# TMElyralab/MuseV

Measured on NVIDIA H100. Metric: denoised frames/sec at 512x512, 16-frame window, 20 DDIM steps, higher is better.
Workload: dtype f16 (fp32 accumulate)

## Files before the change

include/musev_b200.h:

```cpp
#ifndef MUSEV_B200_H_
#define MUSEV_B200_H_

#include <stdint.h>

#ifdef __cplusplus
extern "C" {
#endif

#define MVB_OK 0
#define MVB_ERR_INVALID (-1)
#define MVB_ERR_CUDA (-2)
#define MVB_ERR_STATE (-3)

const char* mvb_last_error(void);
int mvb_version(void);

typedef struct mvb_conv_gemm_desc {
  const void* a0; int c0; long long a0_stride_w, a0_stride_h, a0_stride_n;
  const void* a1; int c1; long long a1_stride_w, a1_stride_h, a1_stride_n;
  int W, H, NF;
  int ntaps; int8_t dy[9]; int8_t dx[9];
  const void* weight; int N;
  void* out; long long ldc;
  const float* bias;
// ... 98 lines not shown
#define MVB_MAX_REFER 16
typedef struct mvb_unet_args {
  const void* sample; int sample_is_f32;
  int B, T, H, W;
  float timestep;
  const void* encoder_hidden_states; int ehs_is_f32; int n_text;
  int has_sample_index;
  int n_vis_cond, vis_cond_first;
  float sample_frame_rate;
  const void* vision_clip_emb; int clip_is_f32; int n_clip; float ip_adapter_scale;
  int n_refer;
  const void* refer_embs[MVB_MAX_REFER]; int refer_t[MVB_MAX_REFER], refer_h[MVB_MAX_REFER], refer_w[MVB_MAX_REFER];
  const void* mid_refer_emb; int mid_refer_t, mid_refer_h, mid_refer_w;
  int refer_is_f32;
  int n_down_residuals;
  const void* down_residuals[MVB_MAX_REFER];
  const void* mid_residual; int residual_is_f32;
  int skip_temporal_layers;
  void* out; int out_is_f32;
  const void* pose_guider_emb; int pose_is_f32;
} mvb_unet_args;

int mvb_create(const mvb_config* cfg, int device, mvb_handle** out);
void mvb_destroy(mvb_handle* h);
int mvb_load_weight(mvb_handle* h, const char* name, const void* device_ptr, int is_f32, const long long* shape, int ndim);
typedef struct mvb_named_tensor {
  const char* name;
  const void* device_ptr;
  int is_f32;
  int ndim;
// ... 78 lines not shown
```

musev_b200/_capi.py:

```python
from __future__ import annotations

import ctypes as C
import hashlib
import os
from types import SimpleNamespace
from typing import Callable, Dict, Iterable, Optional, Sequence, Tuple

import torch
import torch.distributed as dist

from .build import LIB_PATH
from .context import assign_windows

_lib = None


class MvbError(RuntimeError):
    pass


class ConvGemmDesc(C.Structure):
    _fields_ = [
        ("a0", C.c_void_p), ("c0", C.c_int),
        ("a0_stride_w", C.c_longlong), ("a0_stride_h", C.c_longlong), ("a0_stride_n", C.c_longlong),
# ... 40 lines not shown
class MvbUnetArgs(C.Structure):
    _fields_ = [
        ("sample", C.c_void_p), ("sample_is_f32", C.c_int),
        ("B", C.c_int), ("T", C.c_int), ("H", C.c_int), ("W", C.c_int),
        ("timestep", C.c_float),
        ("encoder_hidden_states", C.c_void_p), ("ehs_is_f32", C.c_int), ("n_text", C.c_int),
        ("has_sample_index", C.c_int),
        ("n_vis_cond", C.c_int), ("vis_cond_first", C.c_int),
        ("sample_frame_rate", C.c_float),
        ("vision_clip_emb", C.c_void_p), ("clip_is_f32", C.c_int), ("n_clip", C.c_int), ("ip_adapter_scale", C.c_float),
        ("n_refer", C.c_int),
        ("refer_embs", C.c_void_p * MAX_REFER), ("refer_t", C.c_int * MAX_REFER), ("refer_h", C.c_int * MAX_REFER),
        ("refer_w", C.c_int * MAX_REFER),
        ("mid_refer_emb", C.c_void_p), ("mid_refer_t", C.c_int), ("mid_refer_h", C.c_int), ("mid_refer_w", C.c_int),
        ("refer_is_f32", C.c_int),
        ("n_down_residuals", C.c_int), ("down_residuals", C.c_void_p * MAX_REFER),
        ("mid_residual", C.c_void_p), ("residual_is_f32", C.c_int),
        ("skip_temporal_layers", C.c_int),
        ("out", C.c_void_p), ("out_is_f32", C.c_int),
        ("pose_guider_emb", C.c_void_p), ("pose_is_f32", C.c_int),
    ]


class MvbNamedTensor(C.Structure):
    _fields_ = [("name", C.c_char_p), ("device_ptr", C.c_void_p), ("is_f32", C.c_int), ("ndim", C.c_int),
                ("shape", C.c_longlong * 5)]


MAX_OUT = 13


# ... 375 lines not shown
```

musev_b200/csrc/capi_ops.cu:

```cuda
#include <cuda_runtime.h>
#include <stdint.h>
#include <stdio.h>
#include <string.h>

#include "../../include/musev_b200.h"
#include "attention.cuh"
#include "cond_embed.cuh"
#include "conv_gemm.cuh"
#include "ops.cuh"

using namespace mvb;

static thread_local char g_err[512] = "";

static int fail(const char* what, cudaError_t e) {
  snprintf(g_err, sizeof(g_err), "%s: %s", what ? what : "error", e == cudaSuccess ? "invalid argument" : cudaGetErrorString(e));
  return e == cudaSuccess ? MVB_ERR_INVALID : MVB_ERR_CUDA;
}

static int sm_count() {
  static int n = 0;
  if (!n) {
    int dev = 0;
    if (cudaGetDevice(&dev) != cudaSuccess) return 132;
    if (cudaDeviceGetAttribute(&n, cudaDevAttrMultiProcessorCount, dev) != cudaSuccess || n <= 0) n = 132;
  }
  return n;
}

extern "C" {

const char* mvb_last_error(void) { return g_err; }

int mvb_version(void) { return 6; }

int mvb_op_conv_gemm(const mvb_conv_gemm_desc* d, void* stream) {
  if (!d || !d->a0 || !d->weight || !d->out) return fail("mvb_op_conv_gemm: null pointer", cudaSuccess);
  ASource a0{(const __half*)d->a0, d->c0, d->a0_stride_w, d->a0_stride_h, d->a0_stride_n};
  ASource a1{(const __half*)d->a1, d->c1, d->a1_stride_w, d->a1_stride_h, d->a1_stride_n};
  Epilogue ep;
  ep.out = (__half*)d->out; ep.ldc = d->ldc; ep.bias = d->bias; ep.rowadd = d->rowadd;
  ep.rows_per_group = d->rows_per_group; ep.ld_rowadd = d->ld_rowadd; ep.res = (const __half*)d->residual;
  ep.ld_res = d->ld_res; ep.alpha = d->alpha; ep.beta = d->beta; ep.geglu = d->geglu; ep.act = d->act; ep.out_f32 = d->out_f32;
  const char* err = nullptr;
  if (d->stride2) {
    cudaError_t e2 = launch_conv_s2((cudaStream_t)stream, (const __half*)d->a0, d->c0, d->W, d->H, d->NF,
                                    (const __half*)d->weight, d->N, ep, sm_count(), &err, d->stride2);
    if (e2 != cudaSuccess) return fail(err, e2);
    return MVB_OK;
// ... 48 lines not shown
int mvb_op_temporal_attention(const void* qkv, int ld, int B, int T, int HW, int heads, int d, int dp, float scale,
                              void* out, int ldo, void* stream) {
  cudaError_t e = temporal_attention((cudaStream_t)stream, (const __half*)qkv, ld, B, T, HW, heads, d, dp, scale,
                                     (__half*)out, ldo);
  if (e == cudaErrorInvalidValue)
    return fail("mvb_op_temporal_attention: needs 1 <= T <= 32, d a multiple of 8, dp in {16, 32, 48, 64, 80, 96, 160} "
                "with dp >= d, ld and ldo multiples of 8", cudaSuccess);
  if (e != cudaSuccess) return fail("mvb_op_temporal_attention", e);
  return MVB_OK;
}

int mvb_op_groupnorm(const void* x0, int c0, const void* x1, int c1, int NF, int HW, int groups, int frames_per_stat,
                     float eps, const float* gamma, const float* beta, int silu, void* y, float* scratch, void* stream) {
  int chunks = 0;
  cudaError_t e = gn_stats((cudaStream_t)stream, (const __half*)x0, c0, (const __half*)x1, c1, NF, HW, groups, scratch,
                           &chunks);
  if (e == cudaSuccess)
    e = gn_apply((cudaStream_t)stream, (const __half*)x0, c0, (const __half*)x1, c1, NF, HW, groups, scratch, chunks,
                 frames_per_stat, eps, gamma, beta, silu, (__half*)y);
  if (e != cudaSuccess) return fail("mvb_op_groupnorm", e == cudaErrorInvalidValue ? cudaSuccess : e);
  return MVB_OK;
}

int mvb_op_groupnorm_fused(const void* x0, int c0, const void* x1, int c1, int NF, int HW, int groups, int frames_per_stat,
                           float eps, const float* gamma, const float* beta, int silu, void* y, float* scratch,
                           unsigned int* barrier_word, unsigned int* arrivals, void* stream) {
  if (!barrier_word || !arrivals) return fail("mvb_op_groupnorm_fused: null barrier word", cudaSuccess);
  int dev = 0, sms = 132;
  cudaGetDevice(&dev);
  cudaDeviceGetAttribute(&sms, cudaDevAttrMultiProcessorCount, dev);
  cudaError_t e = gn_fused((cudaStream_t)stream, (const __half*)x0, c0, (const __half*)x1, c1, NF, HW, groups, scratch,
                           frames_per_stat, eps, gamma, beta, silu, (__half*)y, sms, barrier_word, arrivals);
  if (e != cudaSuccess) return fail("mvb_op_groupnorm_fused", e == cudaErrorInvalidValue ? cudaSuccess : e);
  return MVB_OK;
}

int mvb_op_layernorm(const void* x, long long M, int C, float eps, const float* gamma, const float* beta, void* y,
                     void* stream) {
  cudaError_t e = layernorm((cudaStream_t)stream, (const __half*)x, M, C, eps, gamma, beta, (__half*)y);
  if (e != cudaSuccess) return fail("mvb_op_layernorm", e == cudaErrorInvalidValue ? cudaSuccess : e);
  return MVB_OK;
}

int mvb_fuse_cfg_ddim(const float* eps_sum, const float* counter, const void* latents_in, void* latents_out,
                      int is_f32, int B, int C, int T, int HW, int cfg, float guidance_scale, float alpha_prod_t,
                      float alpha_prod_t_prev, int prediction_type, float clip_range, int use_clipped_model_output,
                      float std_dev_t, const float* variance_noise, float* eps_out, float* x0_out, void* stream) {
// ... 54 lines not shown
```

musev_b200/csrc/engine_fwd.cuh:

```cuda
#pragma once
#include <math.h>
#include <stdio.h>

#include <string>

#include "attention.cuh"
#include "conv_gemm.cuh"
#include "engine.cuh"
#include "ops.cuh"

namespace mvb {

inline constexpr const char* kNullArg = "null pointer argument";

struct Engine::Fwd {
  Engine* E;
  Arena* ar;
  cudaStream_t s;
  bool dry;
  int B, T, H, W, NF;
  int heads;
  int groups;
  float gn_eps;
  float* gn_part = nullptr;
  const float* temb_table = nullptr;
  const float* femb_table = nullptr;
  int temb_ld = 0, femb_ld = 0;
  struct Cond {
    const __half* enc = nullptr;
    int n_text = 0;
    const __half* clip = nullptr;
    int n_clip = 0;
    float ip_adapter_scale = 0.f;
    int n_vis_cond = 0, vis_cond_first = 0;
    int refer_is_f32 = 0;
  } cond;
  bool skip_temporal;
  bool ok = true;

  Fwd(Engine* e, Arena& arena, cudaStream_t st, int B_, int T_, int H_, int W_, bool skip_temporal_layers, int groups_,
      float gn_eps_)
      : E(e), ar(&arena), s(st), dry(arena.dry), B(B_), T(T_), H(H_), W(W_), NF(B_ * T_), heads(e->heads_), groups(groups_),
        gn_eps(gn_eps_), skip_temporal(skip_temporal_layers) {
    if (!dry) E->taps_.clear();
    if (groups) gn_part = alloc_f((long long)NF * (kGnMaxChunks + 1) * groups * 2);
  }

  bool fail(const char* what, cudaError_t e) {
    if (ok) {
      char buf[400];
      snprintf(buf, sizeof(buf), "%s: %s", what ? what : "error", e == cudaSuccess ? "failed" : cudaGetErrorString(e));
      E->err_ = buf;
    }
    ok = false;
    return false;
  }
  __half* alloc_h(long long rows, int C) {
    void* p = ar->alloc((size_t)rows * C * sizeof(__half));
    if (!p) fail("workspace too small", cudaSuccess);
    return (__half*)p;
  }
  float* alloc_f(long long n) {
    void* p = ar->alloc((size_t)n * sizeof(float));
    if (!p) fail("workspace too small", cudaSuccess);
    return (float*)p;
  }
  void tap(const std::string& name, const __half* p, long long rows, int C) {
    if (!dry) E->taps_.push_back({name, p, rows, C});
  }
  size_t mark() const { return ar->off; }
  void release(size_t m) { ar->off = m; }

  void gemm_img(const ASource& a0, const ASource* a1, int Wd, int Hd, int NFd, int ntaps, const int8_t* dy,
                const int8_t* dx, const Mat& m, Epilogue ep, bool use_bias = true) {
    if (!ok || dry) return;
    if (use_bias && !ep.bias) ep.bias = m.bias;
    const char* err = nullptr;
    cudaError_t e = launch_conv_gemm(s, a0, a1, Wd, Hd, NFd, ntaps, dy, dx, m.w, m.N, ep, E->num_sms_, &err);
    if (e != cudaSuccess) fail(err, e);
  }
  void gemm(const __half* x, long long M, int K, const Mat& m, Epilogue ep, bool use_bias = true) {
    static const int8_t z = 0;
    ASource a0{x, K, (long long)K, (long long)K * M, (long long)K * M};
// ... 9 lines not shown
  void conv1x1(const __half* x0, int C0, const __half* x1, int C1, long long M, const Mat& m, Epilogue ep) {
    static const int8_t z = 0;
    ASource a0{x0, C0, (long long)C0, (long long)C0 * M, (long long)C0 * M};
    ASource a1{x1, C1, (long long)C1, (long long)C1 * M, (long long)C1 * M};
    gemm_img(a0, x1 ? &a1 : nullptr, (int)M, 1, 1, 1, &z, &z, m, ep);
  }
  void tconv(const __half* x, int C, int HW, const Mat& m, Epilogue ep) {
    static const int8_t dy[3] = {-1, 0, 1}, dx[3] = {0, 0, 0};
    ASource a0{x, C, (long long)C, (long long)C * HW, (long long)C * HW * T};
    gemm_img(a0, nullptr, HW, T, B, 3, dy, dx, m, ep);
  }
  void gn(const __half* x0, int C0, const __half* x1, int C1, int HW, int fps, float eps, const Norm& n, int silu,
          __half* y) {
    if (!gn_part) { fail("groupnorm: the forward reserved no scratch", cudaSuccess); return; }
    if (!ok || dry) return;
    if (E->gn_fused_) {
      cudaError_t e = gn_fused(s, x0, C0, x1, C1, NF, HW, groups, gn_part, fps, eps, n.g, n.b, silu, y,
                               E->num_sms_, E->gn_counter_dev_, &E->gn_base_);
      if (e != cudaSuccess) fail("groupnorm (fused)", e);
      return;
    }
    int chunks = 0;
    cudaError_t e = gn_stats(s, x0, C0, x1, C1, NF, HW, groups, gn_part, &chunks);
    if (e == cudaSuccess)
      e = gn_apply(s, x0, C0, x1, C1, NF, HW, groups, gn_part, chunks, fps, eps, n.g, n.b, silu, y);
    if (e != cudaSuccess) fail("groupnorm", e);
  }
  void ln(const __half* x, long long M, int C, float eps, const Norm& n, __half* y) {
    if (!ok || dry) return;
    cudaError_t e = layernorm(s, x, M, C, eps, n.g, n.b, y);
    if (e != cudaSuccess) fail("layernorm", e);
  }
  void attn(const AttnArgs& aa) {
    if (!ok || dry) return;
    const char* err = nullptr;
    cudaError_t e = launch_attention(s, aa, &err);
    if (e != cudaSuccess) fail(err, e);
  }
// ... 112 lines not shown
  }
  void feed_forward(const TBlock& b, __half* h, long long M, int C, __half* nbuf) {
    const size_t mk = mark();
    ln(h, M, C, E->ln_eps13_, b.n3, nbuf);
    __half* ff = alloc_h(M, 4 * C);
    Epilogue e1;
    e1.out = ff; e1.ldc = 4 * C; e1.geglu = 1;
    gemm(nbuf, M, C, b.ff1, e1);
    Epilogue e2;
    e2.out = h; e2.ldc = C; e2.res = h; e2.ld_res = C;
    gemm(ff, M, 4 * C, b.ff2, e2);
    release(mk);
  }
  __half* spatial(const SpatialT& st, const __half* x, int HW) {
    const int C = st.C, Hh = heads, d = C / Hh, dp = pad16(d), hd = Hh * dp;
    const long long M = (long long)NF * HW;
    __half* out = alloc_h(M, C);
    const size_t mk = mark();
    __half* nbuf = alloc_h(M, C);
    __half* h = alloc_h(M, C);
    gn(x, C, nullptr, 0, HW, 1, 1e-6f, st.norm, 0, nbuf);
    { Epilogue ep; ep.out = h; ep.ldc = C; gemm(nbuf, M, C, st.proj_in, ep); }
    const TBlock& b = st.blk;
    {
      const size_t mk2 = mark();
      ln(h, M, C, E->ln_eps13_, b.n1, nbuf);
      __half* qkv = alloc_h(M, 3 * hd);
      { Epilogue ep; ep.out = qkv; ep.ldc = 3 * hd; gemm(nbuf, M, C, b.qkv1, ep, b.qkv1.bias != nullptr); }
      __half* ao = alloc_h(M, C);
      AttnArgs aa{};
      aa.v_ones_col = b.qkv1.bias != nullptr;
// ... 5 lines not shown
        aa.nseg = 2;
        aa.seg[1] = AttnSegment{qkv + hd, qkv + 2 * hd, 3 * hd, M, cond.n_vis_cond * HW, T, (long long)T * HW,
                                (long long)cond.vis_cond_first * HW};
      }
      aa.out = ao; aa.ldo = C; aa.out_scale = 1.f;
      attn(aa);
      Epilogue ep; ep.out = h; ep.ldc = C; ep.res = h; ep.ld_res = C;
      gemm(ao, M, C, b.out1, ep);
      release(mk2);
    }
    {
      const size_t mk2 = mark();
      ln(h, M, C, 1e-5f, b.n2, nbuf);
      __half* q = alloc_h(M, hd);
      { Epilogue ep; ep.out = q; ep.ldc = hd; gemm(nbuf, M, C, b.q2, ep, false); }
      const long long Mt = (long long)B * cond.n_text;
      __half* kv = alloc_h(Mt, 2 * hd);
      { Epilogue ep; ep.out = kv; ep.ldc = 2 * hd; gemm(cond.enc, Mt, b.kv2.K, b.kv2, ep, b.kv2.bias != nullptr); }
      __half* ao = alloc_h(M, C);
      AttnArgs aa{};
      aa.v_ones_col = b.kv2.bias != nullptr;
      aa.q = q; aa.ldq = hd; aa.NF = NF; aa.Nq = HW; aa.heads = Hh; aa.d = d; aa.dp = dp;
      aa.scale = 1.f / sqrtf((float)d);
      aa.nseg = 1;
      aa.seg[0] = AttnSegment{kv, kv + hd, 2 * hd, Mt, cond.n_text, T, cond.n_text, 0};
      aa.out = ao; aa.ldo = C; aa.out_scale = 1.f;
      attn(aa);
      if (b.has_ip && cond.clip && cond.ip_adapter_scale > 0.f) {
        const long long Mc = (long long)B * cond.n_clip;
        __half* kvi = alloc_h(Mc, 2 * hd);
// ... 66 lines not shown
    AttnArgs aa{};
    aa.q = qkv; aa.ldq = 3 * hd; aa.NF = NF; aa.Nq = HW; aa.heads = Hh; aa.d = d; aa.dp = dp;
    aa.scale = 1.f / sqrtf((float)d);
    aa.nseg = 2;
    aa.v_ones_col = r.qkv.bias != nullptr;
    aa.seg[0] = AttnSegment{kvr, kvr + hd, 2 * hd, Mr, nref, T, nref, 0};
    aa.seg[1] = AttnSegment{qkv + hd, qkv + 2 * hd, 3 * hd, M, HW, 1, HW, 0};
    aa.out = ao; aa.ldo = C; aa.out_scale = 1.f;
    attn(aa);
    Epilogue ep; ep.out = out; ep.ldc = C; ep.res = x; ep.ld_res = C;
    gemm(ao, M, C, r.out, ep);
    release(mk);
    return out;
  }
  __half* refer_tokens(const void* map, int C, int t, int h, int w) {
    __half* tok = alloc_h((long long)B * t * h * w, C);
    if (ok && !dry) {
      cudaError_t e = ncthw_to_tokens(s, map, cond.refer_is_f32, B, C, t, h * w, tok, C, 1.f);
      if (e != cudaSuccess) fail("refer tokens", e);
    }
    return tok;
  }
};

}
```

musev_b200/csrc/engine_unet.cu:

```cuda
#include "engine_fwd.cuh"

namespace mvb {

bool unet_config_ok(const mvb_config* cfg) {
  if (cfg->num_blocks < 1 || cfg->num_blocks > 4 || cfg->heads < 1 || cfg->norm_num_groups < 1) return false;
  for (int i = 0; i < cfg->num_blocks; ++i) {
    const int c = cfg->block_out_channels[i];
    if (c % 64 || c % cfg->heads || (c / cfg->heads) % 8 || c % cfg->norm_num_groups) return false;
  }
  return cfg->cross_attention_dim % 64 == 0 && cfg->in_channels * 9 <= 64;
}

void Engine::build_unet() {
  const mvb_config& c = cfg_;
  UNetWeights& w = model_.emplace<UNetWeights>();
  const int nb = c.num_blocks;
  const int c0 = c.block_out_channels[0], temb = 4 * c0;
  int n_res_c = 0, n_tt_c = 0;
  {
    int ch = c0;
    for (int i = 0; i < nb; ++i) {
      ch = c.block_out_channels[i];
      n_res_c += c.layers_per_block * ch;
      if (i != nb - 1) n_tt_c += c.layers_per_block * ch;
// ... 84 lines not shown
  w.norm_out = make_norm("conv_norm_out", c0);
  w.conv_out = make_mat(16, 9 * c0, true);
  reg_conv_cols("conv_out.weight", w.conv_out, 16, c.out_channels, c0, 9);
  reg_vec("conv_out.bias", w.conv_out.bias, 16, c.out_channels);
}

bool Engine::run_unet(const mvb_unet_args& a, Arena& ar, cudaStream_t s) {
  const mvb_config& c = cfg_;
  const UNetWeights& w = std::get<UNetWeights>(model_);
  const int nb = c.num_blocks, c0 = c.block_out_channels[0], temb = 4 * c0;
  const int B = a.B, T = a.T, NF = a.B * a.T;
  if (a.H % (1 << (nb - 1)) || a.W % (1 << (nb - 1))) { err_ = "H and W must be divisible by 2^(num_blocks-1)"; return false; }
  if (T > 32) { err_ = "at most 32 frames per window (temporal attention kernel)"; return false; }
  if (B < 1 || B > 64 || a.n_vis_cond > 64) { err_ = "batch (incl. CFG) must be in 1..64 and at most 64 vision-condition frames"; return false; }
  if (a.n_vis_cond < 0 || a.vis_cond_first < 0 || a.vis_cond_first + a.n_vis_cond > T) { err_ = "bad vision condition index range"; return false; }
  if (c.need_refer_emb && a.n_refer != 0) {
    int expect = 1;
    for (int i = 0; i < nb; ++i) expect += c.layers_per_block + (i == nb - 1 ? 0 : 1);
    if (a.n_refer != expect) { err_ = "down_block_refer_embs: wrong number of maps"; return false; }
  }
  Fwd f(this, ar, s, B, T, a.H, a.W, a.skip_temporal_layers != 0, c.norm_num_groups, c.norm_eps);

  __half* temb_rows = f.alloc_h(NF, temb);
  __half* femb_rows = f.alloc_h(NF, temb);
  float* temb_table = f.alloc_f((long long)NF * w.temb.rows);
  float* femb_table = f.alloc_f((long long)NF * w.femb.rows);
  f.temb_table = temb_table; f.femb_table = femb_table;
  f.temb_ld = w.temb.rows; f.femb_ld = w.femb.rows;
  {
    const size_t mk = f.mark();
// ... 32 lines not shown
  if (!ar.dry && f.ok) {
    cudaError_t e = ncthw_to_tokens(s, a.encoder_hidden_states, a.ehs_is_f32, 1, 1, 1, B * a.n_text * X, enc, 1, 1.f);
    if (e != cudaSuccess) f.fail("encoder_hidden_states convert", e);
  }
  if (c.ip_adapter_cross_attn && a.vision_clip_emb && a.n_clip > 0) {
    clip = f.alloc_h((long long)B * a.n_clip, X);
    if (!ar.dry && f.ok) {
      cudaError_t e = ncthw_to_tokens(s, a.vision_clip_emb, a.clip_is_f32, 1, 1, 1, B * a.n_clip * X, clip, 1, 1.f);
      if (e != cudaSuccess) f.fail("vision_clip_emb convert", e);
    }
  }
  Fwd::Cond& cd = f.cond;
  cd.enc = enc; cd.n_text = a.n_text; cd.clip = clip; cd.n_clip = a.n_clip; cd.ip_adapter_scale = a.ip_adapter_scale;
  if (c.need_t2i_ip_adapter) { cd.n_vis_cond = a.n_vis_cond; cd.vis_cond_first = a.vis_cond_first; } cd.refer_is_f32 = a.refer_is_f32;

  int Hc = a.H, Wc = a.W;
  const long long M = (long long)NF * Hc * Wc;
  __half* x = f.alloc_h(M, c0);
  f.conv_in(x, a.sample, a.sample_is_f32, c.in_channels, w.conv_in, a.pose_guider_emb, a.pose_is_f32, "conv_in inputs");
  f.tap("conv_in", x, M, c0);
  if (w.has_tin) { x = f.temporal(w.tin, x, Hc * Wc); f.tap("transformer_in", x, M, c0); }
  const bool use_ref = c.need_refer_emb && a.n_refer > 0;
  if (use_ref) {
    __half* tok = f.refer_tokens(a.refer_embs[0], c0, a.refer_t[0], a.refer_h[0], a.refer_w[0]);
    x = f.refer_fuse(w.first_ref, x, Hc * Wc, tok, a.refer_t[0] * a.refer_h[0] * a.refer_w[0]);
    f.tap("first_refer", x, M, c0);
  }
  struct Skip { __half* p; int C, H, W; };
  std::vector<Skip> skips;
  skips.push_back({x, c0, Hc, Wc});
  int ch = c0;
  for (int i = 0; i < nb; ++i) {
    const bool final = i == nb - 1;
    const Block& blk = w.down[i];
    const int num_block = c.layers_per_block + (final ? 0 : 1);
    const int ref_start = 1 + num_block * i;
    for (int j = 0; j < c.layers_per_block; ++j) {
      const Layer& L = blk.layers[j];
      const std::string pn = "down_blocks." + std::to_string(i);
      const long long Ml = (long long)NF * Hc * Wc;
      x = f.resnet(L.res, x, ch, nullptr, 0, Hc, Wc);
      ch = L.res.C;
      f.tap(pn + ".resnets." + std::to_string(j), x, Ml, ch);
      x = f.temp_conv(L.tc, x, Hc * Wc);
      f.tap(pn + ".temp_convs." + std::to_string(j), x, Ml, ch);
      if (L.has_attn) {
        x = f.spatial(L.st, x, Hc * Wc);
        f.tap(pn + ".attentions." + std::to_string(j), x, Ml, ch);
        x = f.temporal(L.tt, x, Hc * Wc);
        f.tap(pn + ".temp_attentions." + std::to_string(j), x, Ml, ch);
      }
      if (use_ref) {
        const int ri = ref_start + j;
        if (ri >= a.n_refer) { err_ = "refer emb index out of range"; return false; }
        __half* tok = f.refer_tokens(a.refer_embs[ri], ch, a.refer_t[ri], a.refer_h[ri], a.refer_w[ri]);
        x = f.refer_fuse(L.ref, x, Hc * Wc, tok, a.refer_t[ri] * a.refer_h[ri] * a.refer_w[ri]);
        f.tap(pn + ".refer_emb_attns." + std::to_string(j), x, Ml, ch);
      }
      skips.push_back({x, ch, Hc, Wc});
    }
    if (!final) {
      x = f.downsample(x, ch, Hc, Wc, blk.sampler, 1);
      Hc /= 2; Wc /= 2;
      if (use_ref) {
        const int ri = ref_start + c.layers_per_block;
        __half* tok = f.refer_tokens(a.refer_embs[ri], ch, a.refer_t[ri], a.refer_h[ri], a.refer_w[ri]);
        x = f.refer_fuse(blk.ref_down, x, Hc * Wc, tok, a.refer_t[ri] * a.refer_h[ri] * a.refer_w[ri]);
      }
      f.tap("down_blocks." + std::to_string(i) + ".down", x, (long long)NF * Hc * Wc, ch);
      skips.push_back({x, ch, Hc, Wc});
    }
  }
  x = f.resnet(w.mid_res[0], x, ch, nullptr, 0, Hc, Wc);
  x = f.temp_conv(w.mid_tc[0], x, Hc * Wc);
  x = f.spatial(w.mid_st, x, Hc * Wc);
  x = f.temporal(w.mid_tt, x, Hc * Wc);
  x = f.resnet(w.mid_res[1], x, ch, nullptr, 0, Hc, Wc);
  x = f.temp_conv(w.mid_tc[1], x, Hc * Wc);
  f.tap("mid", x, (long long)NF * Hc * Wc, ch);
  if (c.need_refer_emb && a.mid_refer_emb) {
    __half* tok = f.refer_tokens(a.mid_refer_emb, ch, a.mid_refer_t, a.mid_refer_h, a.mid_refer_w);
    x = f.refer_fuse(w.mid_ref, x, Hc * Wc, tok, a.mid_refer_t * a.mid_refer_h * a.mid_refer_w);
  }
  if (a.n_down_residuals > 0) {
    if (a.n_down_residuals != (int)skips.size()) { err_ = "down_block_additional_residuals: wrong count"; return false; }
// ... 57 lines not shown
```

musev_b200/csrc/ops.cu:

```cuda
#include "ops.cuh"

#include <math.h>

#include <type_traits>

#include "stats.cuh"

namespace mvb {

__device__ __forceinline__ float silu_f(float x) {
  float e, r;
  asm("ex2.approx.ftz.f32 %0, %1;" : "=f"(e) : "f"(x * -1.4426950408889634f));
  asm("rcp.approx.ftz.f32 %0, %1;" : "=f"(r) : "f"(1.f + e));
  return x * r;
}

struct alignas(16) Half8 {
  __half2 h[4];
};
__device__ __forceinline__ Half8 ld_half8(const __half* p) {
  Half8 r;
  *reinterpret_cast<uint4*>(&r) = __ldg(reinterpret_cast<const uint4*>(p));
  return r;
}
// ... 82 lines not shown
      }
    }
    float* dst = part + ((size_t)f * chunks + chunk) * 2 * G + 2 * g;
    dst[0] = mean;
    dst[1] = m2;
  }
}

__global__ void __launch_bounds__(256, 8)
gn_stats_kernel(const __half* __restrict__ x0, int C0, const __half* __restrict__ x1, int C1, int HW, int G,
                float* __restrict__ part) {
  extern __shared__ float2 spair[];
  gn_stats_unit(x0, C0, x1, C1, HW, G, part, gridDim.y - 1 - blockIdx.y, blockIdx.x, gridDim.x, spair);
}

cudaError_t gn_stats(cudaStream_t s, const __half* x0, int C0, const __half* x1, int C1, int NF, int HW, int G,
                     float* part, int* chunks_out) {
  ProfScope prof(s, KC_GROUPNORM);
  const int C = C0 + (x1 ? C1 : 0);
  if (!x1) C1 = 0;
  if ((C0 % 8) || (C1 % 8) || (C % G) || ((C / G) % 2)) return cudaErrorInvalidValue;
  const int threads = 256;
  int chunks = (8 * 132) / NF;
  const int maxc = HW / 32 > 0 ? HW / 32 : 1;
  if (chunks > maxc) chunks = maxc;
  if (chunks > kGnMaxChunks) chunks = kGnMaxChunks;
  if (chunks < 1) chunks = 1;
  *chunks_out = chunks;
  const int cols = (C / 8) < threads ? (C / 8) : threads;
  const size_t smem = (size_t)(threads / cols) * (C / 2) * sizeof(float2);
  gn_stats_kernel<<<dim3(chunks, NF), threads, smem, s>>>(x0, C0, x1, C1, HW, G, part);
  return cudaGetLastError();
}

__device__ __forceinline__ void gn_finalize_unit(const float* __restrict__ part, int chunks, int fps, int G, int HW, int cpg, float eps,
                                                 float* __restrict__ stats, int sg, int g, int lane) {
  float n = 0.f, mean = 0.f, m2 = 0.f;
  for (int i = lane; i < fps * chunks; i += 32) {
    const int chunk = i % chunks;
    const int pix = (int)(((long long)HW * (chunk + 1)) / chunks) - (int)(((long long)HW * chunk) / chunks);
    const float2 pp = *reinterpret_cast<const float2*>(part + ((size_t)sg * fps * chunks + i) * 2 * G + 2 * g);
    chan_merge(n, mean, m2, (float)pix * (float)cpg, pp.x, pp.y);
// ... 194 lines not shown
  int threads = 256;
  if (vecs <= 256 && (256 % vecs) != 0) threads = (256 / vecs) * vecs;
  if (threads < 64) threads = 256;
  const int rows_per_pass = threads / (vecs < threads ? vecs : threads) > 0 ? threads / (vecs < threads ? vecs : threads) : 1;
  int ppb = (int)(((long long)HW * NF + 132 * 24 - 1) / (132 * 24));
  if (ppb < 4 * rows_per_pass) ppb = 4 * rows_per_pass;
  if (ppb > HW) ppb = HW;
  int blocks = (HW + ppb - 1) / ppb;
  gn_apply_kernel<<<dim3(blocks, NF), threads, 2 * G * sizeof(float), s>>>(x0, C0, x1, C1, HW, G, stats, fps, gamma, beta,
                                                                           silu, y, ppb);
  return cudaGetLastError();
}

cudaError_t gn_fused(cudaStream_t s, const __half* x0, int C0, const __half* x1, int C1, int NF, int HW, int G, float* part,
                     int fps, float eps, const float* gamma, const float* beta, int silu, __half* y, int num_sms,
                     unsigned int* counter, unsigned int* base) {
  ProfScope prof(s, KC_GROUPNORM);
  if (!x1) C1 = 0;
  const int C = C0 + C1;
  if ((C0 % 8) || (C1 % 8) || (C % G) || ((C / G) % 2) || fps < 1 || (NF % fps) || G > 64) return cudaErrorInvalidValue;
  int chunks = (8 * 132) / NF;
  const int maxc = HW / 32 > 0 ? HW / 32 : 1;
  if (chunks > maxc) chunks = maxc;
  if (chunks > kGnMaxChunks) chunks = kGnMaxChunks;
  if (chunks < 1) chunks = 1;
  const int vecs = C / 8;
  int threads = 256;
  if (vecs <= 256 && (256 % vecs) != 0) threads = (256 / vecs) * vecs;
  if (threads < 64) threads = 256;
  const int cols = vecs < threads ? vecs : threads;
  const int rows_per_pass = threads / cols > 0 ? threads / cols : 1;
  int ppb = (int)(((long long)HW * NF + 132 * 24 - 1) / (132 * 24));
  if (ppb < 4 * rows_per_pass) ppb = 4 * rows_per_pass;
  if (ppb > HW) ppb = HW;
  const int pblocks = (HW + ppb - 1) / ppb;
  size_t smem = (size_t)(threads / cols) * (C / 2) * sizeof(float2);
  if (smem < 2 * G * sizeof(float)) smem = 2 * G * sizeof(float);
  int per_sm = 0;
  cudaError_t e = cudaOccupancyMaxActiveBlocksPerMultiprocessor(&per_sm, gn_fused_kernel, threads, smem);
  if (e != cudaSuccess) return e;
// ... 888 lines not shown
```

musev_b200/csrc/ops.cuh:

```cuda
#pragma once
#include <cuda_fp16.h>
#include <cuda_runtime.h>
#include <stdint.h>

namespace mvb {

static constexpr int kGnMaxChunks = 64;

cudaError_t gn_stats(cudaStream_t s, const __half* x0, int C0, const __half* x1, int C1, int NF, int HW, int G,
                     float* part, int* chunks);
cudaError_t gn_apply(cudaStream_t s, const __half* x0, int C0, const __half* x1, int C1, int NF, int HW, int G,
                     const float* part, int chunks, int frames_per_stat, float eps, const float* gamma,
                     const float* beta, int silu, __half* y);
cudaError_t layernorm(cudaStream_t s, const __half* x, long long M, int C, float eps, const float* gamma,
                      const float* beta, __half* y);
cudaError_t upsample2x(cudaStream_t s, const __half* x, int NF, int H, int W, int C, __half* y);
cudaError_t add_tensors(cudaStream_t s, const __half* a, const __half* b, long long n, __half* y);
cudaError_t ncthw_to_tokens(cudaStream_t s, const void* x, int is_f32, int B, int C, int T, int HW, __half* y,
                            int ldy, float scale);
cudaError_t tokens_to_ncthw(cudaStream_t s, const __half* x, int ldx, int B, int C, int T, int HW, void* y,
                            int is_f32);
cudaError_t tokens_to_ncthw_add(cudaStream_t s, const __half* x, int ldx, int B, int C, int T, int HW, void* y,
                                int is_f32);
cudaError_t add_nchw_residual(cudaStream_t s, __half* x, int NF, int C, int HW, const void* r, int is_f32);
cudaError_t im2col_latent(cudaStream_t s, const void* x, int is_f32, int B, int Cin, int T, int H, int W, __half* A);
cudaError_t sinusoid(cudaStream_t s, const float* values, int n, int dim, __half* out, int ld);
cudaError_t expand_rows(cudaStream_t s, const __half* src, int B, int T, int D, const int* zero_t, int nzero, int act,
                        __half* out);
cudaError_t silu_copy(cudaStream_t s, const __half* x, long long n, __half* y);
cudaError_t gn_fused(cudaStream_t s, const __half* x0, int C0, const __half* x1, int C1, int NF, int HW, int G, float* part,
                     int fps, float eps, const float* gamma, const float* beta, int silu, __half* y, int num_sms,
                     unsigned int* counter, unsigned int* base);
cudaError_t latent_pointwise(cudaStream_t s, const void* x, int is_f32, int N, int C, int HW, const float* w, const float* b,
                             float in_scale, float* y);
cudaError_t softmax_rows(cudaStream_t s, __half* x, long long M, int N, long long ld, float scale);
cudaError_t tokens_to_ncthw_affine(cudaStream_t s, const __half* x, int ldx, int B, int C, int T, int HW, void* y, int is_f32,
                                   float alpha, float beta, float lo, float hi);
cudaError_t vae_moments(cudaStream_t s, const float* x, int ldx, int N, int C2, int HW, const float* w, const float* b,
                        int postprocess, float scale, void* y, int is_f32);
cudaError_t temporal_attention(cudaStream_t s, const __half* qkv, int ld, int B, int T, int HW, int heads, int d,
                               int dp, float scale, __half* out, int ldo);
cudaError_t fuse_cfg_ddim(cudaStream_t s, const float* eps_sum, const float* counter, const void* latents_in,
                          void* latents_out, int is_f32, int B, int C, int T, int HW, int cfg, float guidance,
                          float alpha_t, float alpha_prev, int prediction_type, float clip_range, int use_clipped,
                          float std_dev, const float* noise, float* eps_out, float* x0_out);
cudaError_t fuse_cfg_affine(cudaStream_t s, const float* eps_sum, const float* counter, const void* latents_in,
                            void* latents_out, int is_f32, int B, int C, int T, int HW, int cfg, float guidance, float c_x,
// ... 10 lines not shown
```

musev_b200/pipeline.py:

```python
from __future__ import annotations

from dataclasses import dataclass
from typing import Callable, Dict, List, Optional, Sequence, Union

import torch

from . import ops
from .context import assign_windows, prepare_global_context
from .samplers import multistep_update
from .scheduler import DDIMScheduler, _PRED, _variance_noise


@dataclass
class DenoiseOutput:
    latents: torch.Tensor
    windows: List[List[int]]
    windows_per_rank: List[List[int]]


class ParallelDenoiser:
    def __init__(self, unet, scheduler, process_group=None, device_ops=None):
        self.ops = device_ops if device_ops is not None else ops
        self.unet = unet
        self.scheduler = scheduler
        self.pg = process_group
        self._dist = None
        if process_group is not None or (torch.distributed.is_available() and torch.distributed.is_initialized()):
            import torch.distributed as dist
            self._dist = dist
        self.rank = self._dist.get_rank(self.pg) if self._dist else 0
        self.world = self._dist.get_world_size(self.pg) if self._dist else 1

    @torch.no_grad()
    def __call__(
        self,
        latents: torch.Tensor,
        condition_latents: torch.Tensor,
        prompt_embeds: torch.Tensor,
# ... 96 lines not shown
                if pose_guider_emb is not None:
                    ctx = torch.tensor(list(range(n_vc)) + [ci + n_vc for ci in c], dtype=torch.long,
                                       device=pose_guider_emb.device)
                    pe = pose_guider_emb.index_select(2, ctx)
                    if cfg_split:
                        pe = pe[rows]
                    nb, c0, tc = pe.shape[:3]
                    kw["pose_guider_emb"] = pe.permute(0, 2, 1, 3, 4).reshape(nb * tc, c0, h, w)
                if controlnet_fn is not None:
                    if cfg_split:
                        down_res, mid_res = controlnet_fn(c, model_in, t, i, rows)
                    else:
                        down_res, mid_res = controlnet_fn(c, model_in, t, i)
                    kw["down_block_additional_residuals"] = down_res
                    kw["mid_block_additional_residual"] = mid_res
                eps = self.unet(model_in, t, prompt_embeds[rows] if cfg_split else prompt_embeds, sample_index=sub_idx,
                                vision_conditon_frames_sample_index=vis_idx, sample_frame_rate=motion_speed,
                                do_classifier_free_guidance=True, return_dict=False, **kw)[0]
                acc = eps_sum[rows] if cfg_split else eps_sum
                if keep_pos[wi] is None:
                    self.ops.accumulate_window(acc, eps, n_vc, frame_idx_dev[wi])
                else:
                    self.ops.accumulate_window(acc, eps.index_select(2, keep_pos[wi]).contiguous(), 0, frame_idx_dev[wi])
            if self.world > 1:
                self._dist.all_reduce(eps_sum, op=self._dist.ReduceOp.SUM, group=self.pg)
            g = guidance_scale_lst[i] if guidance_scale_lst is not None else guidance_scale
            if is_ddim:
                a_t, a_p, std = sch.step_scalars(t, eta)
                if std > 0.0:
                    latents = self.ops.fuse_cfg_ddim(eps_sum, counter, latents, float(g), a_t, a_p, pred, clip, std_dev=std,
# ... 115 lines not shown
```

musev_b200/unet.py:

```python
from __future__ import annotations

import ctypes as C
from dataclasses import dataclass
from types import SimpleNamespace
from typing import Any, Dict, Optional, Sequence, Tuple, Union

import torch

from ._capi import MAX_REFER, EngineModel, MvbError, MvbNamedTensor, MvbUnetArgs, _is_f32, _named, lib, make_config
from ._capi import MvbConfig, lib as _lib
from .schema import UNetConfig, preset_config, unet_param_shapes


@dataclass
class UNet3DConditionOutput:
    sample: torch.Tensor

    def __getitem__(self, i):
        return (self.sample,)[i]


def check_pose_guider_emb(emb: torch.Tensor, B: int, T: int, c0: int, H: int, W: int) -> None:
    want = (B * T, c0, H, W)
    if tuple(emb.shape) != want:
# ... 65 lines not shown
        sample_frame_rate: int = 10,
        skip_temporal_layers: bool = None,
        frame_index: torch.LongTensor = None,
        down_block_refer_embs: Optional[Tuple[torch.Tensor]] = None,
        mid_block_refer_emb: Optional[torch.Tensor] = None,
        refer_self_attn_emb=None,
        refer_self_attn_emb_mode: str = "read",
        vision_clip_emb: torch.Tensor = None,
        ip_adapter_scale: float = 1.0,
        face_emb: torch.Tensor = None,
        facein_scale: float = 1.0,
        ip_adapter_face_emb: torch.Tensor = None,
        ip_adapter_face_scale: float = 1.0,
        do_classifier_free_guidance: bool = False,
        pose_guider_emb: torch.Tensor = None,
    ):
        self._check_loaded()
        for name, v in (("class_labels", class_labels), ("timestep_cond", timestep_cond), ("attention_mask", attention_mask),
                        ("frame_index", frame_index), ("refer_self_attn_emb", refer_self_attn_emb),
                        ("face_emb", face_emb), ("ip_adapter_face_emb", ip_adapter_face_emb)):
            if v is not None:
                raise NotImplementedError(f"musev_b200: `{name}` is not used by the released presets and is not supported")
        if skip_temporal_layers is not None:
            self.set_skip_temporal_layers(skip_temporal_layers)
        if encoder_hidden_states.ndim != 3:
            raise ValueError(f"only support ndim in [3, 4], but given {encoder_hidden_states.ndim}")
        if vision_condition_frames_sample is not None:
            total = sample.shape[2] + vision_condition_frames_sample.shape[2]
            merged = sample.new_zeros(sample.shape[0], sample.shape[1], total, *sample.shape[3:])
            merged[:, :, sample_index.to(sample.device)] = sample
# ... 49 lines not shown
            for i, r in enumerate(res):
                a.down_residuals[i] = r.data_ptr()
        if mid_block_additional_residual is not None:
            mres = mid_block_additional_residual.to(dev).contiguous()
            if down_block_additional_residuals is not None:
                mres = mres.to(res[0].dtype)
            keep.append(mres)
            a.residual_is_f32 = _is_f32(mres)
            a.mid_residual = mres.data_ptr()
        if pose_guider_emb is not None:
            check_pose_guider_emb(pose_guider_emb, B, T, self.cfg.block_out_channels[0], H, W)
            pose = pose_guider_emb.to(dev).contiguous()
            keep.append(pose)
            a.pose_guider_emb, a.pose_is_f32 = pose.data_ptr(), _is_f32(pose)
        a.skip_temporal_layers = int(self.skip_temporal_layers)
        out = torch.empty((B, self.cfg.out_channels, T, H, W), dtype=sample.dtype, device=dev)
        a.out, a.out_is_f32 = out.data_ptr(), _is_f32(out)
        self._launch(a)
        self._keep = keep
        if skip_temporal_layers is not None:
            self.set_skip_temporal_layers(not skip_temporal_layers)
        if not return_dict:
            return (out,)
        return UNet3DConditionOutput(sample=out)

    __call__ = forward

    def debug_taps(self) -> Dict[str, torch.Tensor]:
        l = lib()
        out = {}
# ... 12 lines not shown
```

Measured before the change: 5.906.

## Share CFG-duplicated UNet prefix by running first layers on half batch

Under classifier-free guidance the conditional and unconditional rows share the same latent sample. The UNet therefore runs its input conv, time-independent prefix and the first spatial block on half the batch, up to the first text cross-attention. Kept buffers are then duplicated into the second half with device copies. Groupnorm chunking is decoupled from NF so the stats layout stays consistent, and the workspace allocations double while halved. This removes redundant compute in the early layers at the cost of extra memcpys and bookkeeping complexity.

```diff
diff --git a/include/musev_b200.h b/include/musev_b200.h
--- a/include/musev_b200.h
+++ b/include/musev_b200.h
@@ -136,6 +136,7 @@
   const void* mid_refer_emb; int mid_refer_t, mid_refer_h, mid_refer_w;
   int refer_is_f32;
   int n_down_residuals;
+  int cfg_shared_sample;
   const void* down_residuals[MVB_MAX_REFER];
   const void* mid_residual; int residual_is_f32;
   int skip_temporal_layers;
diff --git a/musev_b200/_capi.py b/musev_b200/_capi.py
--- a/musev_b200/_capi.py
+++ b/musev_b200/_capi.py
@@ -78,7 +78,7 @@
         ("refer_w", C.c_int * MAX_REFER),
         ("mid_refer_emb", C.c_void_p), ("mid_refer_t", C.c_int), ("mid_refer_h", C.c_int), ("mid_refer_w", C.c_int),
         ("refer_is_f32", C.c_int),
-        ("n_down_residuals", C.c_int), ("down_residuals", C.c_void_p * MAX_REFER),
+        ("n_down_residuals", C.c_int), ("cfg_shared_sample", C.c_int), ("down_residuals", C.c_void_p * MAX_REFER),
         ("mid_residual", C.c_void_p), ("residual_is_f32", C.c_int),
         ("skip_temporal_layers", C.c_int),
         ("out", C.c_void_p), ("out_is_f32", C.c_int),
diff --git a/musev_b200/csrc/capi_ops.cu b/musev_b200/csrc/capi_ops.cu
--- a/musev_b200/csrc/capi_ops.cu
+++ b/musev_b200/csrc/capi_ops.cu
@@ -32,7 +32,7 @@
 
 const char* mvb_last_error(void) { return g_err; }
 
-int mvb_version(void) { return 6; }
+int mvb_version(void) { return 7; }
 
 int mvb_op_conv_gemm(const mvb_conv_gemm_desc* d, void* stream) {
   if (!d || !d->a0 || !d->weight || !d->out) return fail("mvb_op_conv_gemm: null pointer", cudaSuccess);
@@ -111,7 +111,7 @@
                      float eps, const float* gamma, const float* beta, int silu, void* y, float* scratch, void* stream) {
   int chunks = 0;
   cudaError_t e = gn_stats((cudaStream_t)stream, (const __half*)x0, c0, (const __half*)x1, c1, NF, HW, groups, scratch,
-                           &chunks);
+                           &chunks, NF);
   if (e == cudaSuccess)
     e = gn_apply((cudaStream_t)stream, (const __half*)x0, c0, (const __half*)x1, c1, NF, HW, groups, scratch, chunks,
                  frames_per_stat, eps, gamma, beta, silu, (__half*)y);
@@ -127,7 +127,7 @@
   cudaGetDevice(&dev);
   cudaDeviceGetAttribute(&sms, cudaDevAttrMultiProcessorCount, dev);
   cudaError_t e = gn_fused((cudaStream_t)stream, (const __half*)x0, c0, (const __half*)x1, c1, NF, HW, groups, scratch,
-                           frames_per_stat, eps, gamma, beta, silu, (__half*)y, sms, barrier_word, arrivals);
+                           frames_per_stat, eps, gamma, beta, silu, (__half*)y, sms, barrier_word, arrivals, NF);
   if (e != cudaSuccess) return fail("mvb_op_groupnorm_fused", e == cudaErrorInvalidValue ? cudaSuccess : e);
   return MVB_OK;
 }
diff --git a/musev_b200/csrc/engine_fwd.cuh b/musev_b200/csrc/engine_fwd.cuh
--- a/musev_b200/csrc/engine_fwd.cuh
+++ b/musev_b200/csrc/engine_fwd.cuh
@@ -37,6 +37,8 @@
   } cond;
   bool skip_temporal;
   bool ok = true;
+  bool halved = false;
+  std::vector<std::pair<__half*, long long>> halved_keep;
 
   Fwd(Engine* e, Arena& arena, cudaStream_t st, int B_, int T_, int H_, int W_, bool skip_temporal_layers, int groups_,
       float gn_eps_)
@@ -56,17 +58,41 @@
     return false;
   }
   __half* alloc_h(long long rows, int C) {
-    void* p = ar->alloc((size_t)rows * C * sizeof(__half));
+    void* p = ar->alloc((size_t)rows * (halved ? 2 : 1) * C * sizeof(__half));
     if (!p) fail("workspace too small", cudaSuccess);
     return (__half*)p;
   }
   float* alloc_f(long long n) {
-    void* p = ar->alloc((size_t)n * sizeof(float));
+    void* p = ar->alloc((size_t)n * (halved ? 2 : 1) * sizeof(float));
     if (!p) fail("workspace too small", cudaSuccess);
     return (float*)p;
   }
   void tap(const std::string& name, const __half* p, long long rows, int C) {
     if (!dry) E->taps_.push_back({name, p, rows, C});
+    keep(p, rows / 2 * C);
+  }
+  void halve_batch() {
+    B /= 2; NF /= 2;
+    halved = true;
+  }
+  void keep(const __half* p, long long n) {
+    if (!halved) return;
+    for (const auto& k : halved_keep)
+      if (k.first == p) return;
+    halved_keep.push_back({const_cast<__half*>(p), n});
+  }
+  void unhalve_batch() {
+    if (!halved) return;
+    halved = false;
+    B *= 2; NF *= 2;
+    if (!dry)
+      for (const auto& k : halved_keep) {
+        if (!ok) break;
+        cudaError_t e = cudaMemcpyAsync(k.first + k.second, k.first, (size_t)k.second * sizeof(__half),
+                                        cudaMemcpyDeviceToDevice, s);
+        if (e != cudaSuccess) fail("shared prefix: second half copy", e);
+      }
+    halved_keep.clear();
   }
   size_t mark() const { return ar->off; }
   void release(size_t m) { ar->off = m; }
@@ -106,14 +132,15 @@
           __half* y) {
     if (!gn_part) { fail("groupnorm: the forward reserved no scratch", cudaSuccess); return; }
     if (!ok || dry) return;
+    const int chunk_nf = halved ? 2 * NF : NF;
     if (E->gn_fused_) {
       cudaError_t e = gn_fused(s, x0, C0, x1, C1, NF, HW, groups, gn_part, fps, eps, n.g, n.b, silu, y,
-                               E->num_sms_, E->gn_counter_dev_, &E->gn_base_);
+                               E->num_sms_, E->gn_counter_dev_, &E->gn_base_, chunk_nf);
       if (e != cudaSuccess) fail("groupnorm (fused)", e);
       return;
     }
     int chunks = 0;
-    cudaError_t e = gn_stats(s, x0, C0, x1, C1, NF, HW, groups, gn_part, &chunks);
+    cudaError_t e = gn_stats(s, x0, C0, x1, C1, NF, HW, groups, gn_part, &chunks, chunk_nf);
     if (e == cudaSuccess)
       e = gn_apply(s, x0, C0, x1, C1, NF, HW, groups, gn_part, chunks, fps, eps, n.g, n.b, silu, y);
     if (e != cudaSuccess) fail("groupnorm", e);
@@ -256,7 +283,7 @@
   }
   __half* spatial(const SpatialT& st, const __half* x, int HW) {
     const int C = st.C, Hh = heads, d = C / Hh, dp = pad16(d), hd = Hh * dp;
-    const long long M = (long long)NF * HW;
+    long long M = (long long)NF * HW;
     __half* out = alloc_h(M, C);
     const size_t mk = mark();
     __half* nbuf = alloc_h(M, C);
@@ -292,6 +319,11 @@
       ln(h, M, C, 1e-5f, b.n2, nbuf);
       __half* q = alloc_h(M, hd);
       { Epilogue ep; ep.out = q; ep.ldc = hd; gemm(nbuf, M, C, b.q2, ep, false); }
+      if (halved) {
+        keep(x, M * C); keep(h, M * C); keep(q, M * hd);
+        unhalve_batch();
+        M = (long long)NF * HW;
+      }
       const long long Mt = (long long)B * cond.n_text;
       __half* kv = alloc_h(Mt, 2 * hd);
       { Epilogue ep; ep.out = kv; ep.ldc = 2 * hd; gemm(cond.enc, Mt, b.kv2.K, b.kv2, ep, b.kv2.bias != nullptr); }
@@ -388,6 +420,7 @@
     return out;
   }
   __half* refer_tokens(const void* map, int C, int t, int h, int w) {
+    if (halved) { fail("refer_tokens: inside the shared prefix", cudaSuccess); return nullptr; }
     __half* tok = alloc_h((long long)B * t * h * w, C);
     if (ok && !dry) {
       cudaError_t e = ncthw_to_tokens(s, map, cond.refer_is_f32, B, C, t, h * w, tok, C, 1.f);
diff --git a/musev_b200/csrc/engine_unet.cu b/musev_b200/csrc/engine_unet.cu
--- a/musev_b200/csrc/engine_unet.cu
+++ b/musev_b200/csrc/engine_unet.cu
@@ -122,6 +122,7 @@
   if (T > 32) { err_ = "at most 32 frames per window (temporal attention kernel)"; return false; }
   if (B < 1 || B > 64 || a.n_vis_cond > 64) { err_ = "batch (incl. CFG) must be in 1..64 and at most 64 vision-condition frames"; return false; }
   if (a.n_vis_cond < 0 || a.vis_cond_first < 0 || a.vis_cond_first + a.n_vis_cond > T) { err_ = "bad vision condition index range"; return false; }
+  if (a.cfg_shared_sample && B % 2) { err_ = "cfg_shared_sample needs an even batch"; return false; }
   if (c.need_refer_emb && a.n_refer != 0) {
     int expect = 1;
     for (int i = 0; i < nb; ++i) expect += c.layers_per_block + (i == nb - 1 ? 0 : 1);
@@ -184,6 +185,7 @@
   cd.enc = enc; cd.n_text = a.n_text; cd.clip = clip; cd.n_clip = a.n_clip; cd.ip_adapter_scale = a.ip_adapter_scale;
   if (c.need_t2i_ip_adapter) { cd.n_vis_cond = a.n_vis_cond; cd.vis_cond_first = a.vis_cond_first; } cd.refer_is_f32 = a.refer_is_f32;
 
+  if (a.cfg_shared_sample && !a.pose_guider_emb) f.halve_batch();
   int Hc = a.H, Wc = a.W;
   const long long M = (long long)NF * Hc * Wc;
   __half* x = f.alloc_h(M, c0);
@@ -192,6 +194,7 @@
   if (w.has_tin) { x = f.temporal(w.tin, x, Hc * Wc); f.tap("transformer_in", x, M, c0); }
   const bool use_ref = c.need_refer_emb && a.n_refer > 0;
   if (use_ref) {
+    f.unhalve_batch();
     __half* tok = f.refer_tokens(a.refer_embs[0], c0, a.refer_t[0], a.refer_h[0], a.refer_w[0]);
     x = f.refer_fuse(w.first_ref, x, Hc * Wc, tok, a.refer_t[0] * a.refer_h[0] * a.refer_w[0]);
     f.tap("first_refer", x, M, c0);
@@ -199,6 +202,7 @@
   struct Skip { __half* p; int C, H, W; };
   std::vector<Skip> skips;
   skips.push_back({x, c0, Hc, Wc});
+  f.keep(x, (long long)f.NF * Hc * Wc * c0);
   int ch = c0;
   for (int i = 0; i < nb; ++i) {
     const bool final = i == nb - 1;
@@ -228,6 +232,7 @@
         f.tap(pn + ".refer_emb_attns." + std::to_string(j), x, Ml, ch);
       }
       skips.push_back({x, ch, Hc, Wc});
+      f.keep(x, (long long)f.NF * Hc * Wc * ch);
     }
     if (!final) {
       x = f.downsample(x, ch, Hc, Wc, blk.sampler, 1);
@@ -239,6 +244,7 @@
       }
       f.tap("down_blocks." + std::to_string(i) + ".down", x, (long long)NF * Hc * Wc, ch);
       skips.push_back({x, ch, Hc, Wc});
+      f.keep(x, (long long)f.NF * Hc * Wc * ch);
     }
   }
   x = f.resnet(w.mid_res[0], x, ch, nullptr, 0, Hc, Wc);
diff --git a/musev_b200/csrc/ops.cu b/musev_b200/csrc/ops.cu
--- a/musev_b200/csrc/ops.cu
+++ b/musev_b200/csrc/ops.cu
@@ -120,18 +120,23 @@
   gn_stats_unit(x0, C0, x1, C1, HW, G, part, gridDim.y - 1 - blockIdx.y, blockIdx.x, gridDim.x, spair);
 }
 
-cudaError_t gn_stats(cudaStream_t s, const __half* x0, int C0, const __half* x1, int C1, int NF, int HW, int G,
-                     float* part, int* chunks_out) {
-  ProfScope prof(s, KC_GROUPNORM);
-  const int C = C0 + (x1 ? C1 : 0);
-  if (!x1) C1 = 0;
-  if ((C0 % 8) || (C1 % 8) || (C % G) || ((C / G) % 2)) return cudaErrorInvalidValue;
-  const int threads = 256;
-  int chunks = (8 * 132) / NF;
+static int gn_chunks(int chunk_nf, int HW) {
+  int chunks = (8 * 132) / chunk_nf;
   const int maxc = HW / 32 > 0 ? HW / 32 : 1;
   if (chunks > maxc) chunks = maxc;
   if (chunks > kGnMaxChunks) chunks = kGnMaxChunks;
   if (chunks < 1) chunks = 1;
+  return chunks;
+}
+
+cudaError_t gn_stats(cudaStream_t s, const __half* x0, int C0, const __half* x1, int C1, int NF, int HW, int G,
+                     float* part, int* chunks_out, int chunk_nf) {
+  ProfScope prof(s, KC_GROUPNORM);
+  const int C = C0 + (x1 ? C1 : 0);
+  if (!x1) C1 = 0;
+  if ((C0 % 8) || (C1 % 8) || (C % G) || ((C / G) % 2) || chunk_nf < 1) return cudaErrorInvalidValue;
+  const int threads = 256;
+  const int chunks = gn_chunks(chunk_nf, HW);
   *chunks_out = chunks;
   const int cols = (C / 8) < threads ? (C / 8) : threads;
   const size_t smem = (size_t)(threads / cols) * (C / 2) * sizeof(float2);
@@ -356,16 +361,13 @@
 
 cudaError_t gn_fused(cudaStream_t s, const __half* x0, int C0, const __half* x1, int C1, int NF, int HW, int G, float* part,
                      int fps, float eps, const float* gamma, const float* beta, int silu, __half* y, int num_sms,
-                     unsigned int* counter, unsigned int* base) {
+                     unsigned int* counter, unsigned int* base, int chunk_nf) {
   ProfScope prof(s, KC_GROUPNORM);
   if (!x1) C1 = 0;
   const int C = C0 + C1;
-  if ((C0 % 8) || (C1 % 8) || (C % G) || ((C / G) % 2) || fps < 1 || (NF % fps) || G > 64) return cudaErrorInvalidValue;
-  int chunks = (8 * 132) / NF;
-  const int maxc = HW / 32 > 0 ? HW / 32 : 1;
-  if (chunks > maxc) chunks = maxc;
-  if (chunks > kGnMaxChunks) chunks = kGnMaxChunks;
-  if (chunks < 1) chunks = 1;
+  if ((C0 % 8) || (C1 % 8) || (C % G) || ((C / G) % 2) || fps < 1 || (NF % fps) || G > 64 || chunk_nf < 1)
+    return cudaErrorInvalidValue;
+  const int chunks = gn_chunks(chunk_nf, HW);
   const int vecs = C / 8;
   int threads = 256;
   if (vecs <= 256 && (256 % vecs) != 0) threads = (256 / vecs) * vecs;
diff --git a/musev_b200/csrc/ops.cuh b/musev_b200/csrc/ops.cuh
--- a/musev_b200/csrc/ops.cuh
+++ b/musev_b200/csrc/ops.cuh
@@ -8,7 +8,7 @@
 static constexpr int kGnMaxChunks = 64;
 
 cudaError_t gn_stats(cudaStream_t s, const __half* x0, int C0, const __half* x1, int C1, int NF, int HW, int G,
-                     float* part, int* chunks);
+                     float* part, int* chunks, int chunk_nf);
 cudaError_t gn_apply(cudaStream_t s, const __half* x0, int C0, const __half* x1, int C1, int NF, int HW, int G,
                      const float* part, int chunks, int frames_per_stat, float eps, const float* gamma,
                      const float* beta, int silu, __half* y);
@@ -30,7 +30,7 @@
 cudaError_t silu_copy(cudaStream_t s, const __half* x, long long n, __half* y);
 cudaError_t gn_fused(cudaStream_t s, const __half* x0, int C0, const __half* x1, int C1, int NF, int HW, int G, float* part,
                      int fps, float eps, const float* gamma, const float* beta, int silu, __half* y, int num_sms,
-                     unsigned int* counter, unsigned int* base);
+                     unsigned int* counter, unsigned int* base, int chunk_nf);
 cudaError_t latent_pointwise(cudaStream_t s, const void* x, int is_f32, int N, int C, int HW, const float* w, const float* b,
                              float in_scale, float* y);
 cudaError_t softmax_rows(cudaStream_t s, __half* x, long long M, int N, long long ld, float scale);
diff --git a/musev_b200/pipeline.py b/musev_b200/pipeline.py
--- a/musev_b200/pipeline.py
+++ b/musev_b200/pipeline.py
@@ -9,6 +9,7 @@
 from .context import assign_windows, prepare_global_context
 from .samplers import multistep_update
 from .scheduler import DDIMScheduler, _PRED, _variance_noise
+from .unet import UNet3DConditionModel
 
 
 @dataclass
@@ -22,6 +23,7 @@
     def __init__(self, unet, scheduler, process_group=None, device_ops=None):
         self.ops = device_ops if device_ops is not None else ops
         self.unet = unet
+        self._shares_cfg_prefix = isinstance(unet, UNet3DConditionModel)
         self.scheduler = scheduler
         self.pg = process_group
         self._dist = None
@@ -148,6 +150,8 @@
                         down_res, mid_res = controlnet_fn(c, model_in, t, i)
                     kw["down_block_additional_residuals"] = down_res
                     kw["mid_block_additional_residual"] = mid_res
+                if self._shares_cfg_prefix:
+                    kw["cfg_shared_sample"] = not cfg_split
                 eps = self.unet(model_in, t, prompt_embeds[rows] if cfg_split else prompt_embeds, sample_index=sub_idx,
                                 vision_conditon_frames_sample_index=vis_idx, sample_frame_rate=motion_speed,
                                 do_classifier_free_guidance=True, return_dict=False, **kw)[0]
diff --git a/musev_b200/unet.py b/musev_b200/unet.py
--- a/musev_b200/unet.py
+++ b/musev_b200/unet.py
@@ -103,6 +103,7 @@
         ip_adapter_face_scale: float = 1.0,
         do_classifier_free_guidance: bool = False,
         pose_guider_emb: torch.Tensor = None,
+        cfg_shared_sample: bool = False,
     ):
         self._check_loaded()
         for name, v in (("class_labels", class_labels), ("timestep_cond", timestep_cond), ("attention_mask", attention_mask),
@@ -182,6 +183,7 @@
             keep.append(pose)
             a.pose_guider_emb, a.pose_is_f32 = pose.data_ptr(), _is_f32(pose)
         a.skip_temporal_layers = int(self.skip_temporal_layers)
+        a.cfg_shared_sample = int(cfg_shared_sample)
         out = torch.empty((B, self.cfg.out_channels, T, H, W), dtype=sample.dtype, device=dev)
         a.out, a.out_is_f32 = out.data_ptr(), _is_f32(out)
         self._launch(a)
```

After: 6.152, median of 6. 1.04x the previous value.
